# simonsobs/hmvec

Hardware: AMD Instinct MI355X
Metric: (z,m,k) grid-points/sec for P_1h+P_2h (higher is better)
Workload: dtype f64

## Files before the change

### hmvec_amd/csrc/hmctx.hpp

```cpp
#pragma once
#include <hip/hip_runtime.h>
#include <rccl/rccl.h>
#include <rocfft/rocfft.h>

#include <cstdio>
#include <map>
#include <string>
#include <tuple>
#include <vector>

#include "../../include/hmgrid.h"
#include "ldsfft.hpp"
#include "sici.hpp"

extern thread_local std::string g_last_error;
int fail(const char* what, const char* detail, const char* file, int line);
#define HIP_TRY(expr)                                                                   \
    do {                                                                                \
        hipError_t e_ = (expr);                                                         \
        if (e_ != hipSuccess) {                                                         \
            (void)hipGetLastError();                                                    \
            return fail(#expr, hipGetErrorString(e_), __FILE__, __LINE__);              \
        }                                                                               \
    } while (0)
#define FFT_TRY(expr)                                                                   \
    do {                                                                                \
        rocfft_status s_ = (expr);                                                      \
        if (s_ != rocfft_status_success) {                                              \
            char m_[32];                                                                \
            snprintf(m_, sizeof(m_), "rocfft status %d", (int)s_);                      \
            return fail(#expr, m_, __FILE__, __LINE__);                                 \
        }                                                                               \
    } while (0)
#define NCCL_TRY(expr)                                                                  \
    do {                                                                                \
        ncclResult_t r_ = (expr);                                                       \
        if (r_ != ncclSuccess) return fail(#expr, ncclGetErrorString(r_), __FILE__, __LINE__); \
    } while (0)
#define REQUIRE(cond, msg)                                                              \
    do {                                                                                \
        if (!(cond)) return fail("invalid argument", msg, __FILE__, __LINE__);          \
    } while (0)

struct FftPlan {
    rocfft_plan plan = nullptr;
    rocfft_execution_info info = nullptr;
    void* work = nullptr;
    size_t work_bytes = 0;
};

namespace hmg { struct UnpackTw; }
struct FusedPlan {
    hmg::FftPlanDev plan;
    hmg::cplx* twM = nullptr;
    hmg::UnpackTw* twN = nullptr;
    int maxb = 0, maxp = 0;
};

struct PrunedPlan {
    hmg::cplx* twB = nullptr;
    hmg::UnpackTw* twN = nullptr;
    hmg::cplx* twR = nullptr;
    hmg::UnpackTw* twNr = nullptr;
};
struct ChirpPlan {
    hmg::cplx *chP = nullptr, *chJ = nullptr, *Bw = nullptr;
    int Jw = 0;
};
struct SupportKey {
    const void *cmax, *xs, *rss, *ks;
    int rows, nxs, nk;
    long long epoch;
    bool operator<(const SupportKey& o) const {
        return std::tie(cmax, xs, rss, ks, rows, nxs, nk, epoch) < std::tie(o.cmax, o.xs, o.rss, o.ks, o.rows, o.nxs, o.nk, o.epoch);
    }
};

struct PrefixEntry {
    int* nconst = nullptr;
    double* cconst = nullptr;
    int rows = 0, nk = 0;
    bool pending = false;
};

struct hmg_ctx {
    int device = 0;
    hipStream_t stream = nullptr;
    hipStream_t lanes[HMG_LANES] = {};
    int lane = 0;
    hipEvent_t ev[HMG_EVENT_SLOTS] = {};
    int bracket[HMG_KERNEL_COUNT][2];
    void* scratch[7] = {nullptr, nullptr, nullptr, nullptr, nullptr, nullptr, nullptr};
    size_t scratch_bytes[7] = {0, 0, 0, 0, 0, 0, 0};
    std::map<std::pair<int, int>, FftPlan> plans;
    std::map<int, struct FusedPlan> fused;
    size_t fft_chunk_bytes = 0;
    int use_fused_fft = 1;
    int use_pruned_fft = 1;
    int fused_max_m = 6144;
    int fused_prefer_m = 2500;
    int pruned_lp_min = 0;
    int use_chirp = 1;
    int use_band_fft = 1;
    int use_tensor_group = 1;
    int fused_generic = 0;
    int force_gatherv = 0;
    std::map<std::tuple<int, int, int>, ChirpPlan> chirp;
    std::map<std::pair<int, int>, PrunedPlan> pruned;
    std::map<int, hmg::cplx*> pass_tw;
    std::map<SupportKey, std::pair<int, int>> support;
    int* h_fault = nullptr;
    int* d_fault = nullptr;
    long long support_epoch = 0;
    int sig_nz = 0, sig_nm = 0, sig_nq = 0;
    ncclComm_t comm = nullptr;
    int comm_rank = 0, comm_size = 1;
    double* d_barrier = nullptr;
    hmg::SiciTable* d_sici = nullptr;
    void* pinned[2] = {nullptr, nullptr};
    static constexpr int UP_SLOTS = 32;
    static constexpr size_t UP_SLOT_BYTES = (size_t)256 << 10;
    char* up_ring = nullptr;
    hipEvent_t up_ev[UP_SLOTS] = {};
    int up_next = 0;
    hipEvent_t pin_ev[2] = {nullptr, nullptr};
    int num_cu = 256;
    std::multimap<size_t, void*> free_blocks;
    std::map<void*, size_t> block_bytes;
    size_t cached_bytes = 0;
    bool lanes_dirty = false;
    bool capturing = false;
    std::vector<void*> freed_in_capture;
    std::map<int, std::vector<void*>> graph_blocks;
    std::map<int, hipGraphExec_t> graphs;
    std::map<int, int> graph_kernels;
    int next_graph_id = 1;
    int prefix_deferral = 0;
    std::map<void*, PrefixEntry> prefix;
    std::map<void*, PrefixEntry> prefix_capture;
    std::map<int, std::map<void*, PrefixEntry>> graph_prefix;
    hmg_ctx() { for (auto& b : bracket) b[0] = b[1] = -1; }
};
constexpr size_t FREE_CACHE_LIMIT = (size_t)4 << 30;

int event_at(hmg_ctx* c, int slot, hipEvent_t* out);
int check_fault(hmg_ctx* c);
int sync_all(hmg_ctx* c);
int ensure_scratch(hmg_ctx* c, int slot, size_t bytes);
int bracket_open(hmg_ctx* c, int kid, int* stop_slot);
int bracket_close(hmg_ctx* c, int stop_slot);
static inline void prefix_note(hmg_ctx* c, void* out, const PrefixEntry& e) {
    auto& m = c->capturing ? c->prefix_capture : c->prefix;
    if (e.nconst || c->capturing) m[out] = e;
    else m.erase(out);
}
static inline void prefix_replayed(hmg_ctx* c, const std::map<void*, PrefixEntry>& fx) {
    for (auto& kv : fx) {
        if (kv.second.nconst) c->prefix[kv.first] = kv.second;
        else c->prefix.erase(kv.first);
    }
}
static inline void prefix_drop_block(hmg_ctx* c, void* p, size_t bytes) {
    auto lo = c->prefix.lower_bound(p), hi = c->prefix.lower_bound((char*)p + bytes);
    c->prefix.erase(lo, hi);
}
static inline dim3 grid1d(size_t n, int block) { return dim3((unsigned)((n + block - 1) / block)); }
```

### hmvec_amd/csrc/hmgrid.hip

```cpp
#include <algorithm>
#include <cmath>
#include <cstdlib>
#include <cstring>

#include "hmctx.hpp"
#include "fastmath.hpp"
#include "rowdev.hpp"
#include "longgrid.hpp"

#include "kernels/common.hpp"
#include "kernels/sigma2.hpp"
#include "kernels/massfn.hpp"
#include "kernels/halo.hpp"
#include "kernels/nfw.hpp"
#include "kernels/rows.hpp"
#include "kernels/profile_chain.hpp"
#include "kernels/profile_fused.hpp"
#include "kernels/hod.hpp"
#include "kernels/power.hpp"
#include "kernels/power_batch.hpp"
#include "kernels/groups.hpp"
#include "kernels/limber.hpp"
#include "kernels/functions.hpp"

// ... 218 lines not shown
                               double* r200, double* amp, double* xc, double* alpha, double* expo,
                               double* cmax, double* rscale, double* post) {
    REQUIRE(c && ms && cs && rvir && zs && drho1 && rhoc && f && m200 && r200 && amp && xc && alpha && expo &&
                cmax && rscale, "NULL argument");
    RowFit F;
    if (row_fit(kind, hz, post, f, &F)) return 1;
    REQUIRE(nz > 0 && nm > 0, "empty grid");
    RowOut O{amp, xc, alpha, expo, cmax, rscale, post};
    hipLaunchKernelGGL(rows_from_mvir_kernel, grid1d((size_t)nz * nm, 128), dim3(128), 0, c->stream, kind,
                       nz, nm, ms, cs, rvir, zs, drho1, delta2, rhoc, hz, F, gamma, alpha_const, pref,
                       post_pref, m200, r200, O);
    HIP_TRY(hipGetLastError());
    return 0;
}

static int get_plan(hmg_ctx* c, int nxs, int batch, FftPlan** out) {
    auto key = std::make_pair(nxs, batch);
    auto it = c->plans.find(key);
    if (it != c->plans.end()) { *out = &it->second; return 0; }
    REQUIRE(!c->capturing, "a rocFFT plan cannot be created inside a captured step: run the step once eagerly first");
    FftPlan P;
    size_t len = (size_t)nxs;
    FFT_TRY(rocfft_plan_create(&P.plan, rocfft_placement_notinplace, rocfft_transform_type_real_forward,
                               rocfft_precision_double, 1, &len, (size_t)batch, nullptr));
    FFT_TRY(rocfft_plan_get_work_buffer_size(P.plan, &P.work_bytes));
    FFT_TRY(rocfft_execution_info_create(&P.info));
    if (P.work_bytes) {
        HIP_TRY(hipMalloc(&P.work, P.work_bytes));
        FFT_TRY(rocfft_execution_info_set_work_buffer(P.info, P.work, P.work_bytes));
    }
    FFT_TRY(rocfft_execution_info_set_stream(P.info, c->stream));
    auto res = c->plans.emplace(key, P);
    *out = &res.first->second;
    return 0;
}

template <class T>
static int upload_table(const std::vector<T>& h, T** d) {
    HIP_TRY(hipMalloc((void**)d, h.size() * sizeof(T)));
    HIP_TRY(hipMemcpy(*d, h.data(), h.size() * sizeof(T), hipMemcpyHostToDevice));
    return 0;
}

static int fft_chunk(size_t budget, size_t per_row, int rows) {
    const size_t chunk = budget / per_row;
    return chunk < 1 ? 1 : (chunk > (size_t)rows ? rows : (int)chunk);
}
static int fft_r2c(hmg_ctx* c, int n, int nr, double* in, double2* out) {
    FftPlan* P = nullptr;
    if (get_plan(c, n, nr, &P)) return 1;
    void* ib[1] = {in};
    void* ob[1] = {out};
    FFT_TRY(rocfft_execution_info_set_stream(P->info, c->stream));
    FFT_TRY(rocfft_execute(P->plan, ib, ob, P->info));
    return 0;
}


static int get_fused_plan(hmg_ctx* c, int nxs, FusedPlan** out) {
    *out = nullptr;
    auto it = c->fused.find(nxs);
    if (it != c->fused.end()) {
        if (it->second.twM) *out = &it->second;
        return 0;
    }
    FusedPlan P;
    const int M = nxs / 2;
    bool ok = (nxs % 2 == 0) && M >= 4 && fft_make_plan(M, &P.plan) && M <= c->fused_max_m;
    if (ok) {
        int maxb = 0;
        for (int i = 0; i < P.plan.npass; ++i) {
            const int nb = M / P.plan.radix[i];
            maxb = std::max(maxb, (nb + FUSED_NT - 1) / FUSED_NT);
        }
        P.maxb = maxb;
        P.maxp = (M / 2 + FUSED_NT - 1) / FUSED_NT;
        ok = maxb <= 4 && P.maxp <= 8;
    }
    if (!ok) {
        c->fused[nxs] = FusedPlan();
        return 0;
    }
    if (upload_table(pass_tw_table(P.plan), &P.twM) || upload_table(unpack_tw_table(nxs), &P.twN)) return 1;
    auto res = c->fused.emplace(nxs, P);
    *out = &res.first->second;
    return 0;
}

template <class... P, class... Args>
static int launch_lds(void (*kernel)(P...), dim3 grid, dim3 block, size_t lds, hipStream_t stream, const Args&... args) {
    if (lds > 48 * 1024)
        HIP_TRY(hipFuncSetAttribute((const void*)kernel, hipFuncAttributeMaxDynamicSharedMemorySize, (int)lds));
    hipLaunchKernelGGL(kernel, grid, block, lds, stream, args...);
    HIP_TRY(hipGetLastError());
    return 0;
}

template <int B, int P, int S, bool T = false>
struct RowShape {
    static constexpr int MAXB = B, MAXP = P, SPECM = S;
    static constexpr bool TABLE = T;
};
enum Shape { SHAPE_2500, SHAPE_500, SHAPE_1000, SHAPE_1500, SHAPE_2000, SHAPE_3000, SHAPE_RT12, SHAPE_RT23, SHAPE_RT24, SHAPE_RT48 };
template <class F>
static int with_shape(Shape s, F&& f) {
    switch (s) {
        case SHAPE_2500: return f(RowShape<2, 3, 2500, true>{});
        case SHAPE_500: return f(RowShape<1, 1, 500>{});
        case SHAPE_1000: return f(RowShape<1, 1, 1000>{});
        case SHAPE_1500: return f(RowShape<1, 2, 1500>{});
        case SHAPE_2000: return f(RowShape<2, 2, 2000>{});
        case SHAPE_3000: return f(RowShape<3, 3, 3000>{});
        case SHAPE_RT12: return f(RowShape<1, 2, 0>{});
        case SHAPE_RT23: return f(RowShape<2, 3, 0>{});
        case SHAPE_RT24: return f(RowShape<2, 4, 0, true>{});
        case SHAPE_RT48: return f(RowShape<4, 8, 0, true>{});
    }
    return fail("invalid argument", "internal: unknown row shape", __FILE__, __LINE__);
}

static Shape row_shape(const hmg_ctx* c, const FusedPlan& FP, bool table) {
    const FftPlanDev& pl = FP.plan;
    const bool ct = FUSED_NT == 512 && !c->fused_generic;
    if (ct && pl.M == 2500 && pl.npass == 5 && pl.radix[0] == 4 && pl.radix[1] == 5 && pl.radix[2] == 5 &&
        pl.radix[3] == 5 && pl.radix[4] == 5)
        return SHAPE_2500;
    if (table) return FP.maxb <= 2 && FP.maxp <= 4 ? SHAPE_RT24 : SHAPE_RT48;
    if (ct) switch (pl.M) {
            case 500: return SHAPE_500;
            case 1000: return SHAPE_1000;
            case 1500: return SHAPE_1500;
            case 2000: return SHAPE_2000;
            case 3000: return SHAPE_3000;
        }
    if (FP.maxb <= 1 && FP.maxp <= 2) return SHAPE_RT12;
    if (FP.maxb <= 2 && FP.maxp <= 3) return SHAPE_RT23;
    if (FP.maxb <= 2 && FP.maxp <= 4) return SHAPE_RT24;
    return SHAPE_RT48;
}

struct FftRiders {
    const ChainArgs* C = nullptr;
    int nchain = 0;
    size_t chain_lds = 0;
    const NfwArgs* N = nullptr;
    size_t nfw_blocks = 0;
    const double* rho_tab = nullptr;
    int rho_shared = 0;
    bool chain_done = false;
    bool nfw_done = false;
};

struct FftRoute {
    bool xs_aligned = false;
    bool try_long = false;
    FusedPlan* FP = nullptr;
    Shape shape = SHAPE_RT48;
    bool grouped = false;
    bool tensor = false;
};
static int fft_route(hmg_ctx* c, const hmg_profile_fft_part& p, bool chain, bool table, FftRoute* r) {
    *r = FftRoute{};
    r->xs_aligned = p.d_xs && ((uintptr_t)p.d_xs % 16) == 0;
    if (!c->use_fused_fft || !r->xs_aligned) return 0;
    if (get_fused_plan(c, p.nxs, &r->FP)) return 1;
    r->try_long = c->use_pruned_fft && (!r->FP || r->FP->plan.M > c->fused_prefer_m);
// ... 116 lines not shown
    c->support[key] = std::make_pair(h[0], h[1]);
    *p0max = h[0];
    *jnmax = h[1];
    return 0;
}

static int profile_fft_pruned(hmg_ctx* c, const FusedArgs& A0, int rows, bool can_fall_back, int* taken) {
    *taken = 0;
    const int nxs = A0.nxs, M = nxs / 2;
    if ((nxs & 1) || M < 2 * PRUNED_LP[0]) return 0;
    bool any = false;
    for (int lp : PRUNED_LP) any = any || (M % lp == 0 && M / lp >= 2);
    if (!any) return 0;
    int p0max = 0, jnmax = 0, known = 1;
    if (profile_support(c, rows, A0, &p0max, &jnmax, &known)) return 1;
    if (!known) {
        REQUIRE(can_fall_back, "profile support bound unknown inside a captured step: run the step once eagerly first");
        return 0;
    }
    int LP = 0;
    const int lp_min = c->pruned_lp_min > p0max ? c->pruned_lp_min : p0max;
    for (int lp : PRUNED_LP)
        if (M % lp == 0 && M / lp >= 2 && lp >= lp_min) { LP = lp; break; }
    if (!LP)
        for (int lp : PRUNED_LP)
            if (M % lp == 0 && M / lp >= 2 && lp >= p0max) { LP = lp; break; }
    if (!LP) {
        if (!c->use_band_fft || !A0.nconst) return 0;
        int LB = 0;
        for (int lb : {1000, 1024, 1250})
            if (M % lb == 0 && band_lb_compiled(lb) && 2 * jnmax + 2 <= lb) { LB = lb; break; }
        if (!LB) return 0;
        PrunedPlan *PP = nullptr, *PR = nullptr;
        const cplx* twL = nullptr;
        if (get_pruned_plan(c, nxs, 0, &PP)) return 1;
        if (get_pruned_plan(c, nxs, LB, &PR)) return 1;
        if (get_pass_table(c, LB, &twL)) return 1;
        PrunedArgs G{};
        G.F = A0;
        G.F.twN = PP->twN;
        if (ensure_scratch(c, 0, (size_t)3 * nxs * 8)) return 1;
        G.M = M; G.R = M / LB; G.twB = PP->twB; G.twL = twL; G.u = (double*)c->scratch[0]; G.fault = c->d_fault; G.row0 = 0;
        G.twR = PR->twR;
        int stop = -1;
        if (bracket_open(c, HMG_KERNEL_PROFILE_FFT, &stop)) return 1;
        HIP_TRY((hipError_t)launch_band(c->stream, LB, G, rows, jnmax));
        *taken = 1;
        return bracket_close(c, stop);
    }
    PrunedPlan *PP = nullptr, *PR = nullptr;
    const cplx* twL = nullptr;
    if (get_pruned_plan(c, nxs, 0, &PP)) return 1;
    if (get_pruned_plan(c, nxs, LP, &PR)) return 1;
    if (get_pass_table(c, LP, &twL)) return 1;
    size_t rpl = ((size_t)8 << 30) / ((size_t)M * 8);
    if (rpl < 1) rpl = 1;
    if (rpl > (size_t)rows) rpl = rows;
    if (ensure_scratch(c, 0, rpl * (size_t)M * 8)) return 1;
    PrunedArgs G;
    G.F = A0;
    G.F.twN = PP->twN;
    G.M = M; G.R = M / LP; G.twB = PP->twB; G.twL = twL; G.u = (double*)c->scratch[0]; G.fault = c->d_fault; G.row0 = 0;
    G.twR = PR->twR; G.twNr = PR->twNr; G.rmagic = (unsigned)(4294967296ull / (unsigned)G.R) + 1u;
    G.chP = G.chJ = G.Bw = G.twC = nullptr;
    G.Jw = 0; G.p0 = 0;
    if (c->use_chirp && (LP == 1000 || LP == 1250) && p0max >= 1) {
        int p0 = (p0max + 15) / 16 * 16;
        if (p0 > LP) p0 = LP;
        ChirpPlan* CP = nullptr;
        const cplx* twC = nullptr;
        if (get_chirp_plan(c, nxs, LP, p0, &CP)) return 1;
        if (get_pass_table(c, 2 * LP, &twC)) return 1;
        G.chP = CP->chP; G.chJ = CP->chJ; G.Bw = CP->Bw; G.twC = twC; G.Jw = CP->Jw; G.p0 = p0;
    }
    int stop = -1;
    if (bracket_open(c, HMG_KERNEL_PROFILE_FFT, &stop)) return 1;
    HIP_TRY((hipError_t)launch_pruned(c->stream, LP, G, rows, rpl));
    *taken = 1;
    return bracket_close(c, stop);
}

static FusedArgs fused_args(int nm, int nk, const hmg_profile_fft_part& p, const FusedPlan* FP, const FftRiders& R) {
    FusedArgs A{};
    if (FP) { A.plan = FP->plan; A.twM = FP->twM; A.twN = FP->twN; }
    A.nxs = p.nxs; A.nm = nm; A.nk = nk; A.do_norm = p.do_mass_norm;
    A.xs = p.d_xs; A.kts = p.d_kts;
    A.amp = p.d_amp; A.xc = p.d_xc; A.alpha = p.d_alpha; A.expo = p.d_expo;
    A.amp_c = p.amp_const; A.xc_c = p.xc_const; A.alpha_c = p.alpha_const; A.expo_c = p.expo_const; A.gamma = p.gamma;
    A.step = p.fft_step; A.cmax = p.d_cmax; A.rss = p.d_rss; A.zs = p.d_zs; A.ks = p.d_ks; A.post = p.d_post; A.out = p.d_out;
    A.nconst = p.d_nconst; A.cconst = p.d_cconst;
    A.logx = p.d_logxs;
    A.rho_tab = R.rho_tab; A.rho_shared = R.rho_shared;
    A.rowsc = (p.d_rowsc && p.d_nconst) ? p.d_rowsc : nullptr;
    return A;
}

static int profile_fft_impl(hmg_ctx* c, int nz, int nm, int nk, const hmg_profile_fft_part& p, FftRiders& R) {
    const int nxs = p.nxs;
    const double step = p.fft_step;
    const double *xs = p.d_xs, *kts = p.d_kts, *cmax = p.d_cmax, *rss = p.d_rss, *zs = p.d_zs, *ks = p.d_ks;
    R.chain_done = R.nfw_done = false;
    REQUIRE(c && xs && kts && cmax && rss && zs && ks && p.d_out, "NULL argument");
    REQUIRE((p.d_nconst == nullptr) == (p.d_cconst == nullptr), "pass both hint arrays or neither");
    REQUIRE(nz > 0 && nm > 0 && nk > 0, "empty grid");
    prefix_note(c, p.d_out, PrefixEntry{p.d_nconst, p.d_cconst, nz * nm, nk, false});
    REQUIRE(nxs >= 4, "nxs too small");
    const int nh = nxs / 2;
    const int rows = nz * nm;
    REQUIRE(step > 0.0, "step must be positive");
    const bool table = R.rho_tab != nullptr;
    FftRoute r;
    if (fft_route(c, p, R.C && R.nchain > 0, table, &r)) return 1;
    if (r.try_long) {
        int took = 0;
        if (profile_fft_pruned(c, fused_args(nm, nk, p, nullptr, R), rows, r.FP != nullptr, &took)) return 1;
        if (took) return 0;
    }
    if (r.FP) {
        FusedArgs A = fused_args(nm, nk, p, r.FP, R);
        A.defer = c->prefix_deferral && A.nconst;
        int stop = -1;
        if (bracket_open(c, HMG_KERNEL_PROFILE_FFT, &stop)) return 1;
        if (!table && !A.logx && rows >= 8192) {
            if (ensure_scratch(c, 2, (size_t)nxs * 8)) return 1;
            hipLaunchKernelGGL(logx_kernel, grid1d((size_t)nxs, 256), dim3(256), 0, c->stream, nxs, xs,
                               (double*)c->scratch[2]);
            HIP_TRY(hipGetLastError());
            A.logx = (const double*)c->scratch[2];
        }
        int rc;
        if (table) rc = with_shape(r.shape, [&](auto s) { return launch_table<decltype(s)>(c, A, rows); });
        else if (r.grouped) rc = with_shape(r.shape, [&](auto s) { return launch_group<decltype(s)>(c, A, rows, R); });
        else rc = with_shape(r.shape, [&](auto s) { return launch_fused<decltype(s)>(c, A, rows); });
        if (rc) return 1;
        if (A.defer) prefix_note(c, p.d_out, PrefixEntry{A.nconst, A.cconst, rows, nk, true});
        R.chain_done = r.grouped;
        R.nfw_done = r.grouped && R.N;
        return bracket_close(c, stop);
    }
    const int chunk = fft_chunk(c->fft_chunk_bytes ? c->fft_chunk_bytes : ((size_t)160 << 20),
                                (size_t)nxs * 8 + (size_t)(nh + 1) * 16, rows);
    if (ensure_scratch(c, 0, (size_t)chunk * nxs * 8)) return 1;
    if (ensure_scratch(c, 1, (size_t)chunk * (nh + 1) * 16)) return 1;
    if (ensure_scratch(c, 2, (size_t)chunk * 8)) return 1;
    double* fin = (double*)c->scratch[0];
    double2* fout = (double2*)c->scratch[1];
    double* mnorm = (double*)c->scratch[2];
    const bool stage = (size_t)nh * sizeof(double) <= 64 * 1024;
    const size_t lds = stage ? (size_t)nh * sizeof(double) : 0;
    int stop = -1;
    if (!table && bracket_open(c, HMG_KERNEL_PROFILE_FFT, &stop)) return 1;
    for (int r0 = 0; r0 < rows; r0 += chunk) {
        const int nr = rows - r0 < chunk ? rows - r0 : chunk;
        if (table)
            hipLaunchKernelGGL(table_integrand_kernel, dim3(nr), dim3(256), 0, c->stream, nxs, r0, xs, R.rho_tab,
                               R.rho_shared, cmax, p.do_mass_norm, fin, mnorm);
        else
            hipLaunchKernelGGL(integrand_kernel, dim3(nr), dim3(256), 0, c->stream, nxs, r0, xs, p.d_amp, p.d_xc,
                               p.d_alpha, p.d_expo, p.amp_const, p.xc_const, p.alpha_const, p.expo_const, p.gamma, cmax,
                               p.do_mass_norm, (int)r.xs_aligned, fin, mnorm);
        HIP_TRY(hipGetLastError());
        if (fft_r2c(c, nxs, nr, fin, fout)) return 1;
        if (stage)
            hipLaunchKernelGGL(interp_kernel<true>, dim3(nr), dim3(256), lds, c->stream, nm, nk, nh, r0, step,
                               (const double2*)fout, kts, mnorm, rss, zs, ks, p.d_post, p.d_out, p.d_nconst, p.d_cconst);
        else
            hipLaunchKernelGGL(interp_kernel<false>, dim3(nr), dim3(256), 0, c->stream, nm, nk, nh, r0, step,
// ... 685 lines not shown
```

### hmvec_amd/csrc/kernels/profile_fused.hpp

```cpp
#pragma once

namespace hmg {


__global__ void logx_kernel(int n, const double* __restrict__ xs, double* __restrict__ out) {
    const int i = blockIdx.x * blockDim.x + threadIdx.x;
    if (i < n) out[i] = log_fast(xs[i]);
}


template <int NT, int R, int MAXB, bool SMALL = false, int NIN = R, int SRC_SHIFT = 0>
__device__ __forceinline__ void fused_pass(cplx* buf, const cplx* __restrict__ twM, int M, int Ns, int twstep,
                                           unsigned magic, int keep) {
    cplx v[MAXB][R];
    const int nb = M / R;
#pragma unroll
    for (int b = 0; b < MAXB; ++b) {
        const int j = threadIdx.x + b * NT;
        if (j < nb && (keep < 0 || j <= keep || j >= nb - keep)) pass_load<R, SMALL, NIN, SRC_SHIFT>(buf, twM, M, Ns, twstep, magic, j, v[b]);
    }
    __syncthreads();
#pragma unroll
    for (int b = 0; b < MAXB; ++b) {
        const int j = threadIdx.x + b * NT;
// ... 20 lines not shown
#define HMG_FUSED_OCC 8
#endif
#ifndef HMG_RT_OCC
#define HMG_RT_OCC 6
#endif
template <int MAXB, int SPECM> constexpr int fused_occ() { return MAXB > 2 ? 4 : (SPECM ? HMG_FUSED_OCC : HMG_RT_OCC); }
template <int NT, int MAXB, int MAXP, int SPECM, bool TAB = false, bool RSC = false>
__device__ __forceinline__ void profile_fused_row(const FusedArgs& A, int row, double* smem) {
    cplx* buf = reinterpret_cast<cplx*>(smem);
    const int M = SPECM ? SPECM : A.plan.M, nxs = SPECM ? 2 * SPECM : A.nxs;
    double* red = smem + 2 * (size_t)M;
    int* s_cnt = reinterpret_cast<int*>(red + 17);
    const double Aamp = A.amp ? A.amp[row] : A.amp_c;
    const double XC = A.xc ? A.xc[row] : A.xc_c;
    const double AL = A.alpha ? A.alpha[row] : A.alpha_c;
    const double EX = A.expo ? A.expo[row] : A.expo_c;
    const double cm = A.cmax[row];
    const double ln_xc = (TAB || (A.xc == nullptr && A.xc_c == 1.0)) ? 0.0 : log_fast(XC);
    const double* __restrict__ tab = TAB ? A.rho_tab + (A.rho_shared ? (size_t)0 : (size_t)row * (size_t)(SPECM ? 2 * SPECM : A.nxs)) : nullptr;
    const int z = row / A.nm;
    int* s_jn = reinterpret_cast<int*>(red + 18);
    const double* __restrict__ rsc = RSC ? A.rowsc + (size_t)row * HMG_ROWSC_STRIDE : nullptr;
    if (!RSC && threadIdx.x >= NT - 64) {
        const int lane = threadIdx.x & 63;
        const double isc0 = 1.0 / (A.rss[row] * (1.0 + A.zs[z]));
        const double klo0 = A.kts[1] * isc0;
        const double idk0 = 1.0 / klo0;
        int jn0 = M, nleft = 0;
        if (A.nconst) {
            const double tmax = A.ks[A.nk - 1] * idk0;
            if (tmax < (double)(M - 4)) jn0 = (int)tmax + 3;
            int base = 0, end = A.nk;
            for (;;) {
                const int stp = (end - base + 63) >> 6;
                const int first = base + lane * stp;
                bool below = false;
                if (first < end) {
                    const int last = first + stp - 1;
                    below = A.ks[last < end ? last : end - 1] < klo0;
                }
                base += __popcll(__ballot(below)) * stp;
                if (base >= end) { base = end; break; }
                if (stp == 1) break;
                end = base + stp < end ? base + stp : end;
            }
            nleft = base;
        }
        if (lane == 0) {
            *s_cnt = nleft;
            *s_jn = jn0;
            red[19] = isc0; red[20] = klo0; red[21] = A.kts[M] * isc0; red[22] = idk0;
            red[23] = 1.0 / A.kts[1];
        }
    }
    const int R0 = SPECM ? fused_first_radix<SPECM>() : A.plan.radix[0];
    const int stride0 = M / R0;
    const bool pruned = (SPECM || A.plan.npass > 1) && A.xs[2 * stride0] > cm;
    const bool lead3 = SPECM == 2500 && pruned && A.xs[2 * 375] > cm;
    const int pend = lead3 ? 375 : (pruned ? stride0 : M);
    double acc = 0.0;
    for (int p = threadIdx.x; p < pend; p += NT) {
        const int j = 2 * p;
        const double2 xv = *reinterpret_cast<const double2*>(A.xs + j);
        double r0 = 0.0, r1 = 0.0;
        if constexpr (TAB) {
            if (!(fabs(xv.x) > cm)) r0 = tab[j];
            if (!(fabs(xv.y) > cm)) r1 = tab[j + 1];
        } else {
            if (!(fabs(xv.x) > cm)) r0 = gnfw_rho_fast((A.logx ? A.logx[j] : log_fast(xv.x)) - ln_xc, Aamp, AL, EX, A.gamma);
            if (!(fabs(xv.y) > cm)) r1 = gnfw_rho_fast((A.logx ? A.logx[j + 1] : log_fast(xv.y)) - ln_xc, Aamp, AL, EX, A.gamma);
        }
        const cplx y = cplx{xv.x * r0, xv.y * r1};
        if (pruned && SPECM != 2500) {
            const int rot = (threadIdx.x >> 2);
            for (int t = 0; t < R0; ++t) buf[R0 * p + (t + rot) % R0] = y;
        } else {
            buf[p] = y;
        }
        if (A.do_norm && (r0 != 0.0 || r1 != 0.0)) {
            const double xl = (j > 0) ? A.xs[j - 1] : xv.x, xr = (j + 2 < nxs) ? A.xs[j + 2] : xv.y;
            acc += 0.5 * (xv.y - xl) * (r0 * (xv.x * xv.x)) + 0.5 * (xr - xv.x) * (r1 * (xv.y * xv.y));
        }
    }
    {
        const double ws = wave_sum(acc);
        if ((threadIdx.x & 63) == 0) red[threadIdx.x >> 6] = ws;
        __syncthreads();
    }
    if (threadIdx.x < 64) {
        double tot = red[0];
#pragma unroll
        for (int w = 1; w < NT / 64; ++w) tot += red[w];
        const double mnorm = A.do_norm ? tot : 1.0;
        if (threadIdx.x == 0) red[24] = -A.step / mnorm * (RSC ? rsc[4] : red[23]);
    }
    const int jn = RSC ? __double2hiint(rsc[5]) : __builtin_amdgcn_readfirstlane(*s_jn);
    if constexpr (SPECM == 2500) {
        constexpr unsigned mg4 = small_magic(4), mg20 = small_magic(20), mg100 = small_magic(100), mg500 = small_magic(500);
        if (!pruned) fused_pass<NT, 4, MAXB, true>(buf, A.twM, 2500, 1, 1, 0u, -1);
        if (pruned) {
            if (lead3) fused_pass<NT, 5, 1, true, 3, 2>(buf, A.twM + 1, 2500, 4, 1, mg4, -1);
            else fused_pass<NT, 5, 1, true, 5, 2>(buf, A.twM + 1, 2500, 4, 1, mg4, -1);
        } else fused_pass<NT, 5, 1, true>(buf, A.twM + 1, 2500, 4, 1, mg4, -1);
        fused_pass<NT, 5, 1, true>(buf, A.twM + 5, 2500, 20, 1, mg20, -1);
        fused_pass<NT, 5, 1, true>(buf, A.twM + 25, 2500, 100, 1, mg100, -1);
        fused_pass<NT, 5, 1, true>(buf, A.twM + 125, 2500, 500, 1, mg500, 2 * jn + 2 < 500 ? jn : -1);
    } else if constexpr (SPECM != 0) {
        fused_passes_ct<NT, SPECM, 0>(buf, A.twM, pruned, jn);
    } else
    for (int ps = pruned ? 1 : 0; ps < A.plan.npass; ++ps) {
        const int R = A.plan.radix[ps], Ns = A.plan.ns[ps], tws = 1;
        const unsigned mg = A.plan.magic[ps];
        const cplx* __restrict__ twp = A.twM + A.plan.twoff[ps];
        const bool one = (M / R) <= NT;
        const int keep = (ps == A.plan.npass - 1 && 2 * jn + 2 < M / R) ? jn : -1;
        if (R == 5) { if (one) fused_pass<NT, 5, 1>(buf, twp, M, Ns, tws, mg, keep); else fused_pass<NT, 5, MAXB>(buf, twp, M, Ns, tws, mg, keep); }
        else if (R == 4) { if (one) fused_pass<NT, 4, 1>(buf, twp, M, Ns, tws, mg, keep); else fused_pass<NT, 4, MAXB>(buf, twp, M, Ns, tws, mg, keep); }
        else if (R == 3) { if (one) fused_pass<NT, 3, 1>(buf, twp, M, Ns, tws, mg, keep); else fused_pass<NT, 3, MAXB>(buf, twp, M, Ns, tws, mg, keep); }
        else { if (one) fused_pass<NT, 2, 1>(buf, twp, M, Ns, tws, mg, keep); else fused_pass<NT, 2, MAXB>(buf, twp, M, Ns, tws, mg, keep); }
    }
    const double sc = red[24];
    double ua[MAXP], ub[MAXP];
    const int half = M / 2;
#pragma unroll
    for (int b = 0; b < MAXP; ++b) {
        const int j = 1 + threadIdx.x + b * NT;
        const bool hi = (M - j <= jn);
        if (j <= half && (j <= jn || hi)) {
            const cplx zj = buf[j], zmj = buf[M - j];
            const UnpackTw w = A.twN[j];
            double fa, fb;
            unpack_imag_pair(zj, zmj, w.co, w.si, fa, fb);
            ua[b] = fa * sc * w.rj;
            ub[b] = hi ? fb * sc * w.rmj : 0.0;
        }
    }
    __syncthreads();
    double* u = smem;
#pragma unroll
    for (int b = 0; b < MAXP; ++b) {
        const int j = 1 + threadIdx.x + b * NT;
        const bool hi = (M - j <= jn);
        if (j <= half && (j <= jn || hi)) {
            u[j - 1] = ua[b];
            if (hi && M - j >= 1) u[M - j - 1] = ub[b];
        }
    }
    if (threadIdx.x == 0) u[M - 1] = 0.0;
    __syncthreads();
    const double k_lo = RSC ? rsc[1] : red[20], k_hi = RSC ? rsc[2] : red[21], inv_dk = RSC ? rsc[3] : red[22];
    const double pf = A.post ? A.post[row] : 1.0;
    const double u1 = u[0];
    double* __restrict__ dst = A.out + (size_t)row * A.nk;
    const int nleft = RSC ? __double2loint(rsc[5]) : (A.nconst ? __builtin_amdgcn_readfirstlane(*s_cnt) : 0);
    if (nleft > 0) {
        typedef double v2d __attribute__((ext_vector_type(2)));
        const double c = u1 * pf;
        const int nskip = A.defer ? (nleft & ~(HMG_PREFIX_TILE - 1)) : 0;
        double* __restrict__ d0 = dst + nskip;
        const int nfill = nleft - nskip;
        const int head = (int)((reinterpret_cast<uintptr_t>(d0) >> 3) & 1);
        const int npair = (nfill - head) >> 1;
        v2d* __restrict__ d2 = reinterpret_cast<v2d*>(d0 + head);
        const v2d cc = {c, c};
        for (int q = threadIdx.x; q < npair; q += NT) __builtin_nontemporal_store(cc, &d2[q]);
        if (threadIdx.x == 0 && nfill > 0) {
            if (head) __builtin_nontemporal_store(c, &d0[0]);
            if ((nfill - head) & 1) __builtin_nontemporal_store(c, &d0[nfill - 1]);
        }
    }
    auto interp = [&](double k) {
        int j = (int)(k * inv_dk);
        j = j < 1 ? 1 : (j > M - 1 ? M - 1 : j);
        const double fr = fma(k, inv_dk, -(double)j);
        const double y0 = u[j - 1], y1 = u[j];
        return fma(y1 - y0, fr, y0);
    };
    if (A.nconst) {
        for (int i = (nleft & ~63) + threadIdx.x; i < A.nk; i += NT) {
            if (i < nleft) continue;
            const double k = A.ks[i];
            const double val = k > k_hi ? 0.0 : interp(k);
            __builtin_nontemporal_store(val * pf, &dst[i]);
        }
    } else {
        for (int i = threadIdx.x; i < A.nk; i += NT) {
            const double k = A.ks[i];
            const double val = k < k_lo ? u1 : (k > k_hi ? 0.0 : interp(k));
            __builtin_nontemporal_store(val * pf, &dst[i]);
        }
    }
    if (A.nconst && threadIdx.x == 0) {
        A.nconst[row] = nleft;
        A.cconst[row] = u1 * pf;
    }
}
template <int NT, int MAXB, int MAXP, int SPECM>
__global__ __launch_bounds__(NT, (fused_occ<MAXB, SPECM>())) void profile_fused_kernel(FusedArgs A) {
    extern __shared__ __attribute__((aligned(16))) double smem[];
    profile_fused_row<NT, MAXB, MAXP, SPECM>(A, blockIdx.x, smem);
}
template <int NT, int MAXB, int MAXP, int SPECM>
__global__ __launch_bounds__(NT, (fused_occ<MAXB, SPECM>())) void profile_table_kernel(FusedArgs A) {
    extern __shared__ __attribute__((aligned(16))) double smem[];
    profile_fused_row<NT, MAXB, MAXP, SPECM, true>(A, blockIdx.x, smem);
}

__global__ __launch_bounds__(256) void prefix_fill_kernel(int nk, const int* __restrict__ nconst,
                                                          const double* __restrict__ cconst, double* __restrict__ out) {
    typedef double v2d __attribute__((ext_vector_type(2)));
    const int row = blockIdx.x;
    int n = nconst[row] & ~(HMG_PREFIX_TILE - 1);
    n = n < nk ? n : nk;
    if (n <= 0) return;
    const double c = cconst[row];
    double* __restrict__ dst = out + (size_t)row * nk;
    const int head = (int)((reinterpret_cast<uintptr_t>(dst) >> 3) & 1);
    const int npair = (n - head) >> 1;
    v2d* __restrict__ d2 = reinterpret_cast<v2d*>(dst + head);
    const v2d cc = {c, c};
    for (int q = threadIdx.x; q < npair; q += 256) __builtin_nontemporal_store(cc, &d2[q]);
    if (threadIdx.x == 0) {
        if (head) __builtin_nontemporal_store(c, &dst[0]);
        if ((n - head) & 1) __builtin_nontemporal_store(c, &dst[n - 1]);
    }
}


}
```

### hmvec_amd/csrc/ldsfft.hpp

```cpp
#pragma once

#include <vector>
#if defined(__HIPCC__)
#include <hip/hip_runtime.h>
#define HMG_HD __host__ __device__ __forceinline__
#else
#define HMG_HD inline
#endif

namespace hmg {

struct alignas(16) cplx {
    double x, y;
};
HMG_HD cplx cmul(cplx a, cplx b) { return {a.x * b.x - a.y * b.y, a.x * b.y + a.y * b.x}; }
HMG_HD cplx cadd(cplx a, cplx b) { return {a.x + b.x, a.y + b.y}; }
HMG_HD cplx csub(cplx a, cplx b) { return {a.x - b.x, a.y - b.y}; }
HMG_HD cplx cmul_mi(cplx a) { return {a.y, -a.x}; }

constexpr int FFT_MAX_PASSES = 16;
struct FftPlanDev {
    int M;
    int npass;
    int radix[FFT_MAX_PASSES];
    int ns[FFT_MAX_PASSES];
    int twstep[FFT_MAX_PASSES];
    unsigned magic[FFT_MAX_PASSES];
    int twoff[FFT_MAX_PASSES];
};

HMG_HD unsigned fast_div(unsigned j, unsigned magic) {
#if defined(__HIP_DEVICE_COMPILE__)
    return magic ? __umulhi(j, magic) : j;
#else
    return magic ? (unsigned)(((unsigned long long)j * magic) >> 32) : j;
#endif
}

HMG_HD unsigned mul_small(unsigned a, unsigned b) {
#if defined(__HIP_DEVICE_COMPILE__)
    return __umul24(a, b);
#else
    return a * b;
#endif
}
constexpr unsigned small_magic(unsigned d) { return d == 1 ? 0u : ((1u << 20) + d - 1) / d; }
template <bool SMALL>
HMG_HD unsigned div_ns(unsigned j, unsigned magic) {
    if constexpr (SMALL) return magic ? mul_small(j, magic) >> 20 : j;
    else return fast_div(j, magic);
}
template <bool SMALL>
HMG_HD int mul_idx(int a, int b) {
    if constexpr (SMALL) return (int)mul_small((unsigned)a, (unsigned)b);
    else return a * b;
}

constexpr bool fft_plan_fill(int M, FftPlanDev& p) {
    p.M = M;
    p.npass = 0;
    int rem = M;
    const int cand[4] = {5, 4, 3, 2};
    for (int ci = 0; ci < 4; ++ci) {
        const int r = cand[ci];
        while (rem % r == 0 && rem > 1) {
            if (p.npass >= FFT_MAX_PASSES) return false;
            p.radix[p.npass++] = r;
            rem /= r;
        }
    }
    for (int i = 1; i < p.npass; ++i)
        for (int j = i; j > 0 && p.radix[j - 1] > p.radix[j]; --j) {
            const int tmp = p.radix[j];
            p.radix[j] = p.radix[j - 1];
            p.radix[j - 1] = tmp;
        }
    if (p.npass >= 3 && (p.radix[0] == 2 || p.radix[0] == 4) && (p.radix[1] == 2 || p.radix[1] == 4)) {
        for (int i = 2; i < p.npass; ++i)
            if (p.radix[i] == 5) {
                for (int j = i; j > 1; --j) p.radix[j] = p.radix[j - 1];
                p.radix[1] = 5;
                break;
            }
    }
// ... 271 lines not shown
    const long long r = (n * n) % (2LL * M);
    const long double ang = 3.14159265358979323846264338327950288L * (long double)r / (long double)M;
    return cplx{(double)cosl(ang), (double)-sinl(ang)};
}
struct ldc { long double re, im; };
inline void ld_dft(const ldc* x, int n, int stride, ldc* out, const ldc* tw, int N) {
    if (n == 1) { out[0] = x[0]; return; }
    int p = 2;
    while (n % p) ++p;
    const int m = n / p;
    std::vector<ldc> sub((size_t)n);
    for (int r = 0; r < p; ++r) ld_dft(x + (size_t)r * stride, m, stride * p, sub.data() + (size_t)r * m, tw, N);
    const int step = N / n;
    for (int q = 0; q < p; ++q)
        for (int k = 0; k < m; ++k) {
            long double sr = 0.0L, si = 0.0L;
            const long long kk = (long long)k + (long long)q * m;
            for (int r = 0; r < p; ++r) {
                const ldc w = tw[(size_t)((r * kk) % n) * step];
                const ldc y = sub[(size_t)r * m + k];
                sr += y.re * w.re - y.im * w.im;
                si += y.re * w.im + y.im * w.re;
            }
            out[kk] = ldc{sr, si};
        }
}
inline ChirpTables chirp_make_tables(int M, int Lc, int P0, int nwin = 0) {
    ChirpTables T;
    T.M = M; T.Lc = Lc; T.P0 = P0;
    T.Jw = (Lc - P0) / 2;
    T.Kp = Lc - P0 + 1;
    if (T.Jw > M / 2 - 1) T.Jw = M / 2 - 1;
    while (nwin > 0 && T.Jw + nwin * T.Kp > M / 2 - 1) --nwin;
    T.nwin = nwin;
    T.chP.resize(Lc / 2);
    for (int p = 0; p < Lc / 2; ++p) T.chP[p] = chirp_value(p, M);
    const int jmax = T.Jw + nwin * T.Kp;
    T.chJ.resize(jmax + 1);
    for (int j = 0; j <= jmax; ++j) T.chJ[j] = chirp_value(j, M);
    const long double pi = 3.14159265358979323846264338327950288L;
    std::vector<ldc> tw((size_t)Lc), b((size_t)Lc), B((size_t)Lc);
    for (int t = 0; t < Lc; ++t) tw[t] = ldc{cosl(2 * pi * t / Lc), -sinl(2 * pi * t / Lc)};
    auto g = [&](long long n) {
        const long long r = (n * n) % (2LL * M);
        const long double ang = pi * (long double)r / (long double)M;
        return ldc{cosl(ang), sinl(ang)};
    };
    auto emit = [&]() {
        ld_dft(b.data(), Lc, 1, B.data(), tw.data(), Lc);
        for (int k = 0; k < Lc; ++k) T.Bw.push_back(cplx{(double)(B[k].re / Lc), (double)(B[k].im / Lc)});
    };
    for (int m = 0; m < Lc; ++m) b[m] = ldc{0.0L, 0.0L};
    for (int n = 0; n <= T.Jw; ++n) b[n] = g(n);
    for (int n = 1; n <= T.Jw + P0 - 1; ++n) b[Lc - n] = g(-n);
    emit();
    for (int w = 1; w <= nwin; ++w) {
        const long long j0 = T.Jw + 1 + (long long)(w - 1) * T.Kp;
        for (int m = 0; m < Lc; ++m) b[m] = g(j0 - (P0 - 1) + m);
        emit();
        for (int m = 0; m < Lc; ++m) b[m] = g(j0 + T.Kp - 1 + (P0 - 1) - m);
        emit();
    }
    return T;
}
HMG_HD void chirp_first_pass(cplx z0, cplx z1, cplx c0, cplx c1, cplx* v) {
    const cplx a0 = cmul(z0, c0), a1 = cmul(z1, c1);
    v[0] = cadd(a0, a1);
    v[1] = cadd(a0, cmul_mi(a1));
    v[2] = csub(a0, a1);
    v[3] = csub(a0, cmul_mi(a1));
}
HMG_HD cplx chirp_plus(const cplx* Y, int Kp, int j0, int j, cplx chj) { return cmul(chj, Y[Kp - (j - j0)]); }
HMG_HD cplx chirp_minus(const cplx* Y, int j0, int j, cplx chj) { return cmul(chj, Y[1 + (j - j0)]); }
HMG_HD double chirp_unpack(const cplx* Y, int Lc, int j, cplx chj, const UnpackTw& w) {
    const cplx zj = cmul(chj, Y[Lc - j]), zmj = cmul(chj, Y[j]);
    double fa, fb;
    unpack_imag_pair(zj, zmj, w.co, w.si, fa, fb);
    return fa;
}

HMG_HD int band_mode(int t, int jn) { return t - jn; }
HMG_HD int band_index(int j, int LB) { return j < 0 ? LB + j : j; }

}
```

### hmvec_amd/csrc/rowdev.hpp

```cpp
#pragma once
#include <hip/hip_runtime.h>

#include "fastmath.hpp"
#include "ldsfft.hpp"

#ifndef HMG_FUSED_NT
#define HMG_FUSED_NT 512
#endif

namespace hmg {

constexpr int FUSED_NT = HMG_FUSED_NT;

constexpr int WAVE = 64;

template <int CTRL, int ROW_MASK>
__device__ __forceinline__ double dpp_move(double v) {
    const int lo = __builtin_amdgcn_update_dpp(0, __double2loint(v), CTRL, ROW_MASK, 0xf, false);
    const int hi = __builtin_amdgcn_update_dpp(0, __double2hiint(v), CTRL, ROW_MASK, 0xf, false);
    return __hiloint2double(hi, lo);
}
__device__ __forceinline__ double wave_sum(double v) {
    v += dpp_move<0xB1, 0xf>(v);
    v += dpp_move<0x4E, 0xf>(v);
    v += dpp_move<0x141, 0xf>(v);
    v += dpp_move<0x140, 0xf>(v);
    v += dpp_move<0x142, 0xa>(v);
    v += dpp_move<0x143, 0xc>(v);
    return __hiloint2double(__builtin_amdgcn_readlane(__double2hiint(v), 63),
                            __builtin_amdgcn_readlane(__double2loint(v), 63));
}

struct FusedArgs {
    FftPlanDev plan;
    int nxs, nm, nk, do_norm;
    const double* xs;
    const cplx* twM;
    const UnpackTw* twN;
    const double* kts;
    const double *amp, *xc, *alpha, *expo;
    double amp_c, xc_c, alpha_c, expo_c, gamma, step;
    const double *cmax, *rss, *zs, *ks, *post;
    double* out;
    int* nconst;
    double* cconst;
    const double* logx;
    const double* rho_tab;
    int rho_shared;
    int defer;
    const double* rowsc;
};

__device__ __forceinline__ double gnfw_rho_fast(double lt , double A, double AL, double EX,
                                                double gamma) {
    const double ta = exp_fast<false>(fmin(AL * lt, 700.0));
    return A * exp_fast<false>(gamma * lt - EX * log1p_abs(ta));
}

__device__ __forceinline__ double gnfw_rho_alpha1(double lt , double t , double A, double EX,
                                                  double gamma) {
    return A * exp_fast<false>(gamma * lt - EX * log1p_abs(t));
}

}
```

### hmvec_amd/csrc/runtime.hip

```cpp
#include <algorithm>
#include <cmath>
#include <cstdlib>
#include <cstring>

#include "hmctx.hpp"

using namespace hmg;

thread_local std::string g_last_error;

int fail(const char* what, const char* detail, const char* file, int line) {
    char buf[512];
    snprintf(buf, sizeof(buf), "%s: %s (%s:%d)", what, detail, file, line);
    g_last_error = buf;
    return 1;
}

static int rocfft_refcount = 0;

int event_at(hmg_ctx* c, int slot, hipEvent_t* out) {
    if (!c->ev[slot]) HIP_TRY(hipEventCreate(&c->ev[slot]));
    *out = c->ev[slot];
    return 0;
}

int check_fault(hmg_ctx* c) {
    if (!*(volatile int*)c->h_fault) return 0;
    *(volatile int*)c->h_fault = 0;
    c->support.clear();
    return fail("device fault", "a profile row's support exceeded the bound its launch was sized for (the rows were "
                "filled with NaN); the cached bound is dropped - run the step eagerly again", __FILE__, __LINE__);
}
int sync_all(hmg_ctx* c) {
    REQUIRE(!c->capturing, "this call synchronises the device and cannot be part of a captured step");
    for (auto& st : c->lanes) HIP_TRY(hipStreamSynchronize(st));
    c->lanes_dirty = false;
    return check_fault(c);
}

int ensure_scratch(hmg_ctx* c, int slot, size_t bytes) {
    if (c->scratch_bytes[slot] >= bytes) return 0;
    REQUIRE(!c->capturing, "scratch must not grow inside a captured step: run the step once eagerly first");
    if (c->scratch[slot]) {
        if (sync_all(c)) return 1;
        HIP_TRY(hipFree(c->scratch[slot]));
        c->scratch[slot] = nullptr;
        c->scratch_bytes[slot] = 0;
    }
    size_t want = bytes + bytes / 8;
    HIP_TRY(hipMalloc(&c->scratch[slot], want));
    c->scratch_bytes[slot] = want;
    return 0;
}


int hmg_abi_version(void) { return HMG_ABI_VERSION; }
const char* hmg_last_error(void) { return g_last_error.c_str(); }

static int ctx_init(hmg_ctx* c, int device) {
    c->device = device;
    hipDeviceProp_t prop;
    HIP_TRY(hipGetDeviceProperties(&prop, device));
    c->num_cu = prop.multiProcessorCount;
    {
        int lo = 0, hi = 0;
        HIP_TRY(hipDeviceGetStreamPriorityRange(&lo, &hi));
        for (int i = 0; i < HMG_LANES; ++i)
            HIP_TRY(hipStreamCreateWithPriority(&c->lanes[i], hipStreamNonBlocking, i == 0 ? hi : lo));
    }
    c->stream = c->lanes[0];
    {
        const hmg::SiciTable t = hmg::sici_table_host();
        HIP_TRY(hipMalloc((void**)&c->d_sici, sizeof(t)));
        HIP_TRY(hipMemcpy(c->d_sici, &t, sizeof(t), hipMemcpyHostToDevice));
    }
    if (const char* s = getenv("HMG_FUSED_FFT")) c->use_fused_fft = atoi(s);
    if (const char* s = getenv("HMG_PRUNED_FFT")) c->use_pruned_fft = atoi(s);
    if (const char* s = getenv("HMG_FUSED_MAX_M")) c->fused_max_m = atoi(s);
    if (const char* s = getenv("HMG_FUSED_PREFER_M")) c->fused_prefer_m = atoi(s);
    if (const char* s = getenv("HMG_PRUNED_LP_MIN")) c->pruned_lp_min = atoi(s);
    if (const char* s = getenv("HMG_CHIRP")) c->use_chirp = atoi(s);
    if (const char* s = getenv("HMG_BAND_FFT")) c->use_band_fft = atoi(s);
    if (const char* s = getenv("HMG_NO_TENSOR_GROUP")) c->use_tensor_group = !atoi(s);
    if (getenv("HMG_FUSED_GENERIC")) c->fused_generic = 1;
    if (const char* s = getenv("HMG_FORCE_GATHERV")) c->force_gatherv = atoi(s);
    HIP_TRY(hipHostMalloc((void**)&c->h_fault, 64, hipHostMallocMapped | hipHostMallocCoherent));
    *c->h_fault = 0;
    HIP_TRY(hipHostGetDevicePointer((void**)&c->d_fault, c->h_fault, 0));
    if (const char* s = getenv("HMG_FFT_CHUNK_MB")) c->fft_chunk_bytes = (size_t)atol(s) << 20;
    return 0;
}

int hmg_ctx_create(int device, hmg_ctx** out) {
    REQUIRE(out != nullptr, "out is NULL");
    int ndev = 0;
    HIP_TRY(hipGetDeviceCount(&ndev));
    REQUIRE(ndev > 0, "no HIP device visible");
    REQUIRE(device >= 0 && device < ndev, "device index out of range");
    HIP_TRY(hipSetDevice(device));
    if (rocfft_refcount == 0) FFT_TRY(rocfft_setup());
    ++rocfft_refcount;
    hmg_ctx* c = new hmg_ctx();
    if (ctx_init(c, device)) {
        const std::string keep = g_last_error;
        hmg_ctx_destroy(c);
        g_last_error = keep;
        return 1;
    }
    *out = c;
    return 0;
}

int hmg_ctx_destroy(hmg_ctx* c) {
    if (!c) return 0;
    (void)hipSetDevice(c->device);
    for (auto& st : c->lanes) if (st) (void)hipStreamSynchronize(st);
    if (c->comm) { ncclCommDestroy(c->comm); c->comm = nullptr; }
    for (auto& kv : c->graphs) (void)hipGraphExecDestroy(kv.second);
    for (auto& kv : c->plans) {
        if (kv.second.info) rocfft_execution_info_destroy(kv.second.info);
        if (kv.second.plan) rocfft_plan_destroy(kv.second.plan);
        if (kv.second.work) (void)hipFree(kv.second.work);
    }
    for (auto& kv : c->fused) {
        if (kv.second.twM) (void)hipFree(kv.second.twM);
        if (kv.second.twN) (void)hipFree(kv.second.twN);
    }
    for (auto& kv : c->chirp) {
        if (kv.second.chP) (void)hipFree(kv.second.chP);
        if (kv.second.chJ) (void)hipFree(kv.second.chJ);
        if (kv.second.Bw) (void)hipFree(kv.second.Bw);
    }
    for (auto& kv : c->pruned) {
        if (kv.second.twB) (void)hipFree(kv.second.twB);
        if (kv.second.twN) (void)hipFree(kv.second.twN);
        if (kv.second.twR) (void)hipFree(kv.second.twR);
        if (kv.second.twNr) (void)hipFree(kv.second.twNr);
    }
    for (auto& kv : c->pass_tw) (void)hipFree(kv.second);
    if (c->h_fault) (void)hipHostFree(c->h_fault);
    for (auto& s : c->scratch) if (s) (void)hipFree(s);
    for (auto& kv : c->free_blocks) (void)hipFree(kv.second);
    for (auto& kv : c->graph_blocks)
        for (void* p : kv.second) (void)hipFree(p);
    for (void* p : c->freed_in_capture) (void)hipFree(p);
    if (c->d_barrier) (void)hipFree(c->d_barrier);
    if (c->d_sici) (void)hipFree(c->d_sici);
    if (c->up_ring) {
        (void)hipHostFree(c->up_ring);
        for (auto& e : c->up_ev) if (e) (void)hipEventDestroy(e);
    }
    for (int i = 0; i < 2; ++i) {
        if (c->pinned[i]) (void)hipHostFree(c->pinned[i]);
        if (c->pin_ev[i]) (void)hipEventDestroy(c->pin_ev[i]);
    }
    for (auto& e : c->ev) if (e) (void)hipEventDestroy(e);
    for (auto& st : c->lanes) if (st) (void)hipStreamDestroy(st);
    if (--rocfft_refcount == 0) rocfft_cleanup();
    delete c;
    return 0;
}

int hmg_malloc(hmg_ctx* c, size_t bytes, void** d_out) {
    REQUIRE(c && d_out, "NULL argument");
    if (!bytes) bytes = 8;
    REQUIRE(!c->capturing, "device allocation inside a captured step: run the step once eagerly first");
    auto it = c->free_blocks.find(bytes);
    if (it != c->free_blocks.end()) {
        *d_out = it->second;
        c->cached_bytes -= bytes;
        c->free_blocks.erase(it);
        return 0;
    }
    HIP_TRY(hipSetDevice(c->device));
    hipError_t e = hipMalloc(d_out, bytes);
    if (e != hipSuccess && !c->free_blocks.empty()) {
        if (sync_all(c)) return 1;
        for (auto& kv : c->free_blocks) { (void)hipFree(kv.second); c->block_bytes.erase(kv.second); }
        c->free_blocks.clear();
        c->cached_bytes = 0;
        e = hipMalloc(d_out, bytes);
    }
    HIP_TRY(e);
    c->block_bytes[*d_out] = bytes;
    return 0;
}
int hmg_free(hmg_ctx* c, void* p) {
    REQUIRE(c, "NULL ctx");
    if (!p) return 0;
    auto it = c->block_bytes.find(p);
    REQUIRE(it != c->block_bytes.end(), "pointer was not allocated by hmg_malloc of this context");
    if (c->capturing) {
        c->freed_in_capture.push_back(p);
        return 0;
    }
    if (c->lanes_dirty && sync_all(c)) return 1;
    const size_t bytes = it->second;
    prefix_drop_block(c, p, bytes);
    if (c->cached_bytes + bytes <= FREE_CACHE_LIMIT) {
        c->free_blocks.emplace(bytes, p);
        c->cached_bytes += bytes;
        return 0;
    }
    if (sync_all(c)) return 1;
    HIP_TRY(hipFree(p));
    c->block_bytes.erase(it);
    return 0;
}
int hmg_host_alloc(hmg_ctx* c, size_t bytes, void** h_out) {
// ... 265 lines not shown
```

Baseline: 858.6 billion.

## Replace FFT with direct MFMA sine transform for short-support profile rows

For the nxs=5000 fused profile kernel, when the input is nonzero only in a short leading window and few output modes are needed (jn up to a threshold), it computes the sine transform directly. It does this as a dense matrix product using FP64 MFMA instructions against a precomputed cos/sin table, instead of running the full 2500-point LDS FFT passes. This targets FFT work that is wasted when support and mode count are small. The cost is a per-plan twiddle table in global memory, extra table reads per tile, and a specialised path that applies only for SPECM=2500/NT=512 with constant prefixes.

```diff
diff --git a/hmvec_amd/csrc/hmctx.hpp b/hmvec_amd/csrc/hmctx.hpp
--- a/hmvec_amd/csrc/hmctx.hpp
+++ b/hmvec_amd/csrc/hmctx.hpp
@@ -54,6 +54,8 @@
     hmg::FftPlanDev plan;
     hmg::cplx* twM = nullptr;
     hmg::UnpackTw* twN = nullptr;
+    double* dsT = nullptr;
+    int ds_jd = 0;
     int maxb = 0, maxp = 0;
 };
 
@@ -101,6 +103,7 @@
     int fused_prefer_m = 2500;
     int pruned_lp_min = 0;
     int use_chirp = 1;
+    int direct_jd = 128;
     int use_band_fft = 1;
     int use_tensor_group = 1;
     int fused_generic = 0;
diff --git a/hmvec_amd/csrc/hmgrid.hip b/hmvec_amd/csrc/hmgrid.hip
--- a/hmvec_amd/csrc/hmgrid.hip
+++ b/hmvec_amd/csrc/hmgrid.hip
@@ -324,6 +324,10 @@
         return 0;
     }
     if (upload_table(pass_tw_table(P.plan), &P.twM) || upload_table(unpack_tw_table(nxs), &P.twN)) return 1;
+    if (nxs == 5000 && c->direct_jd > 0) {
+        P.ds_jd = std::min(c->direct_jd, (int)DS_JD_MAX);
+        if (upload_table(direct_sine_table(nxs, P.ds_jd), &P.dsT)) return 1;
+    }
     auto res = c->fused.emplace(nxs, P);
     *out = &res.first->second;
     return 0;
@@ -606,7 +610,7 @@
 
 static FusedArgs fused_args(int nm, int nk, const hmg_profile_fft_part& p, const FusedPlan* FP, const FftRiders& R) {
     FusedArgs A{};
-    if (FP) { A.plan = FP->plan; A.twM = FP->twM; A.twN = FP->twN; }
+    if (FP) { A.plan = FP->plan; A.twM = FP->twM; A.twN = FP->twN; A.dsT = FP->dsT; A.ds_jd = FP->ds_jd; }
     A.nxs = p.nxs; A.nm = nm; A.nk = nk; A.do_norm = p.do_mass_norm;
     A.xs = p.d_xs; A.kts = p.d_kts;
     A.amp = p.d_amp; A.xc = p.d_xc; A.alpha = p.d_alpha; A.expo = p.d_expo;
diff --git a/hmvec_amd/csrc/kernels/profile_fused.hpp b/hmvec_amd/csrc/kernels/profile_fused.hpp
--- a/hmvec_amd/csrc/kernels/profile_fused.hpp
+++ b/hmvec_amd/csrc/kernels/profile_fused.hpp
@@ -126,6 +126,7 @@
             acc += 0.5 * (xv.y - xl) * (r0 * (xv.x * xv.x)) + 0.5 * (xr - xv.x) * (r1 * (xv.y * xv.y));
         }
     }
+    if (lead3 && threadIdx.x >= 375 && threadIdx.x < DS_SPAN / 2) buf[threadIdx.x] = cplx{0.0, 0.0};
     {
         const double ws = wave_sum(acc);
         if ((threadIdx.x & 63) == 0) red[threadIdx.x >> 6] = ws;
@@ -139,6 +140,34 @@
         if (threadIdx.x == 0) red[24] = -A.step / mnorm * (RSC ? rsc[4] : red[23]);
     }
     const int jn = RSC ? __double2hiint(rsc[5]) : __builtin_amdgcn_readfirstlane(*s_jn);
+    bool direct = false;
+    if constexpr (SPECM == 2500 && NT == 512)
+        direct = lead3 && A.nconst && A.dsT && direct_sine_takes(2 * 375, jn, A.ds_jd);
+    if (direct) {
+        typedef double ds_d4 __attribute__((ext_vector_type(4)));
+        const int lane = threadIdx.x & 63, wv = threadIdx.x >> 6, ntile = direct_sine_tiles(jn);
+        const double* __restrict__ ya = smem + direct_sine_sample(0, lane);
+        double* stage = smem + DS_SPAN;
+#pragma unroll 1
+        for (int t = wv; t < ntile; t += NT / 64) {
+            const double* __restrict__ tile = A.dsT + (size_t)t * DS_TILE;
+            ds_d4 P = {0.0, 0.0, 0.0, 0.0}, Q = {0.0, 0.0, 0.0, 0.0};
+#pragma unroll 4
+            for (int s = 0; s < DS_KSTEPS; ++s) {
+                const double a = ya[4 * s];
+                P = __builtin_amdgcn_mfma_f64_16x16x4f64(a, tile[direct_sine_k_index(0, s, lane)], P, 0, 0, 0);
+                Q = __builtin_amdgcn_mfma_f64_16x16x4f64(a, tile[direct_sine_k_index(1, s, lane)], Q, 0, 0, 0);
+            }
+            const double p[4] = {P[0], P[1], P[2], P[3]}, qq[4] = {Q[0], Q[1], Q[2], Q[3]};
+            const double w = direct_sine_lane_sum(tile, lane, p, qq);
+            const ds_d4 S = __builtin_amdgcn_mfma_f64_16x16x4f64(1.0, w, ds_d4{0.0, 0.0, 0.0, 0.0}, 0, 0, 0);
+            if (lane < 16) stage[16 * t + lane] = S[0];
+        }
+        __syncthreads();
+        const int j = 1 + threadIdx.x;
+        if (j <= 16 * ntile) smem[j - 1] = stage[j - 1] * red[24] * A.twN[j].rj;
+        __syncthreads();
+    } else {
     if constexpr (SPECM == 2500) {
         constexpr unsigned mg4 = small_magic(4), mg20 = small_magic(20), mg100 = small_magic(100), mg500 = small_magic(500);
         if (!pruned) fused_pass<NT, 4, MAXB, true>(buf, A.twM, 2500, 1, 1, 0u, -1);
@@ -190,8 +219,10 @@
             if (hi && M - j >= 1) u[M - j - 1] = ub[b];
         }
     }
-    if (threadIdx.x == 0) u[M - 1] = 0.0;
+    if (threadIdx.x == 0) smem[M - 1] = 0.0;
     __syncthreads();
+    }
+    double* u = smem;
     const double k_lo = RSC ? rsc[1] : red[20], k_hi = RSC ? rsc[2] : red[21], inv_dk = RSC ? rsc[3] : red[22];
     const double pf = A.post ? A.post[row] : 1.0;
     const double u1 = u[0];
diff --git a/hmvec_amd/csrc/ldsfft.hpp b/hmvec_amd/csrc/ldsfft.hpp
--- a/hmvec_amd/csrc/ldsfft.hpp
+++ b/hmvec_amd/csrc/ldsfft.hpp
@@ -1,5 +1,6 @@
 #pragma once
 
+#include <cmath>
 #include <vector>
 #if defined(__HIPCC__)
 #include <hip/hip_runtime.h>
@@ -437,4 +438,47 @@
 HMG_HD int band_mode(int t, int jn) { return t - jn; }
 HMG_HD int band_index(int j, int LB) { return j < 0 ? LB + j : j; }
 
-}
+constexpr int DS_LS = 48, DS_NSEG = 16, DS_SPAN = DS_LS * DS_NSEG, DS_KSTEPS = DS_LS / 4;
+constexpr int DS_TILE_K = 2 * DS_KSTEPS * 64, DS_TILE = DS_TILE_K + 2 * 4 * 64;
+constexpr int DS_MAXT = 4;
+constexpr int DS_JD_MAX = 16 * DS_MAXT * 8;
+HMG_HD int direct_sine_tiles(int jn) { return (jn + 15) >> 4; }
+HMG_HD bool direct_sine_takes(int zero_from, int jn, int jd) { return jd > 0 && zero_from <= DS_SPAN && jn >= 1 && jn <= jd; }
+HMG_HD int direct_sine_sample(int s, int lane) { return DS_LS * (lane & 15) + 4 * s + (lane >> 4); }
+HMG_HD int direct_sine_k_index(int tab, int s, int lane) { return (tab * DS_KSTEPS + s) * 64 + lane; }
+HMG_HD int direct_sine_seg_index(int tab, int reg, int lane) { return DS_TILE_K + (tab * 4 + reg) * 64 + lane; }
+HMG_HD double direct_sine_lane_sum(const double* tile, int lane, const double* p, const double* q) {
+    double w = 0.0;
+#if defined(__HIP_DEVICE_COMPILE__)
+#pragma unroll
+#endif
+    for (int reg = 0; reg < 4; ++reg) {
+        w = fma(tile[direct_sine_seg_index(0, reg, lane)], p[reg], w);
+        w = fma(tile[direct_sine_seg_index(1, reg, lane)], q[reg], w);
+    }
+    return w;
+}
+inline std::vector<double> direct_sine_table(int nxs, int jd) {
+    const int nt = direct_sine_tiles(jd);
+    std::vector<double> t((size_t)nt * DS_TILE);
+    const long double twopi = 6.283185307179586476925286766559L;
+    auto ang = [&](long long j, long long n) { return twopi * (long double)((j * n) % nxs) / (long double)nxs; };
+    for (int ti = 0; ti < nt; ++ti)
+        for (int lane = 0; lane < 64; ++lane) {
+            const int j = 16 * ti + 1 + (lane & 15);
+            double* tile = t.data() + (size_t)ti * DS_TILE;
+            for (int s = 0; s < DS_KSTEPS; ++s) {
+                const long double a = ang(j, 4 * s + (lane >> 4));
+                tile[direct_sine_k_index(0, s, lane)] = (double)cosl(a);
+                tile[direct_sine_k_index(1, s, lane)] = (double)sinl(a);
+            }
+            for (int reg = 0; reg < 4; ++reg) {
+                const long double a = ang(j, (long long)DS_LS * ((lane >> 4) + 4 * reg));
+                tile[direct_sine_seg_index(0, reg, lane)] = (double)-sinl(a);
+                tile[direct_sine_seg_index(1, reg, lane)] = (double)-cosl(a);
+            }
+        }
+    return t;
+}
+
+}
diff --git a/hmvec_amd/csrc/rowdev.hpp b/hmvec_amd/csrc/rowdev.hpp
--- a/hmvec_amd/csrc/rowdev.hpp
+++ b/hmvec_amd/csrc/rowdev.hpp
@@ -49,6 +49,8 @@
     int rho_shared;
     int defer;
     const double* rowsc;
+    const double* dsT;
+    int ds_jd;
 };
 
 __device__ __forceinline__ double gnfw_rho_fast(double lt , double A, double AL, double EX,
diff --git a/hmvec_amd/csrc/runtime.hip b/hmvec_amd/csrc/runtime.hip
--- a/hmvec_amd/csrc/runtime.hip
+++ b/hmvec_amd/csrc/runtime.hip
@@ -80,6 +80,7 @@
     if (const char* s = getenv("HMG_FUSED_PREFER_M")) c->fused_prefer_m = atoi(s);
     if (const char* s = getenv("HMG_PRUNED_LP_MIN")) c->pruned_lp_min = atoi(s);
     if (const char* s = getenv("HMG_CHIRP")) c->use_chirp = atoi(s);
+    if (const char* s = getenv("HMG_DIRECT_SINE")) c->direct_jd = std::min(std::max(atoi(s), 0), (int)hmg::DS_JD_MAX);
     if (const char* s = getenv("HMG_BAND_FFT")) c->use_band_fft = atoi(s);
     if (const char* s = getenv("HMG_NO_TENSOR_GROUP")) c->use_tensor_group = !atoi(s);
     if (getenv("HMG_FUSED_GENERIC")) c->fused_generic = 1;
@@ -125,6 +126,7 @@
     for (auto& kv : c->fused) {
         if (kv.second.twM) (void)hipFree(kv.second.twM);
         if (kv.second.twN) (void)hipFree(kv.second.twN);
+        if (kv.second.dsT) (void)hipFree(kv.second.dsT);
     }
     for (auto& kv : c->chirp) {
         if (kv.second.chP) (void)hipFree(kv.second.chP);
```

Result: slower. 837.5 billion (-2.5%).
